# haan6/fm-for-online-recommendation

Measured on AMD Instinct MI355X. Metric: samples/sec online-FM (Criteo-39-field, k=16) FTRL-proximal, higher is better.
Workload: dtype f32

## Files before the change

### fm-for-online-recommendation_amd/csrc/fmx_common.h

```cpp
#pragma once
#include <hip/hip_runtime.h>
#include <hip/hip_ext.h>

#include <cstdarg>
#include <cstdio>
#include <cstdlib>
#include <cstring>
#include <atomic>
#include <mutex>

#include "fmx.h"

#pragma clang fp contract(off)

namespace fmxd {
extern thread_local char g_err[512];
int fail(int code, const char *fmt, ...);
int check_launch(const char *what);

struct Tune {
  int wpb_fwd = 4, wpb_upd = 2;
  int sort_e = 0;
  int inline_fixup = 1;
  int online_persistent = 1;
  int afm_online_persistent = 1;
  int afm_pair_online_persistent = 1;
  int sort_ahead = 16;
  int mlp_chain = 1;
  int sort_chunked = 1;
};
Tune &tune();

constexpr int FMX_COMM_SLOTS = 4;
struct Comm {
  int rank = 0, world = 1, n_blocks = 1;
  bool force = false;
  int block_count[FMX_COMM_MAX_WORLD] = {0}, block_first[FMX_COMM_MAX_WORLD] = {0};
  void *main = nullptr, *pf = nullptr;
  hipStream_t pf_stream = nullptr;
  hipEvent_t fork = nullptr, ready[FMX_COMM_SLOTS] = {nullptr}, free_[FMX_COMM_SLOTS] = {nullptr};
  bool used[FMX_COMM_SLOTS] = {false};
};
int comm_all_gather(Comm *c, int which, const void *send, void *recv, size_t count, hipStream_t st);
int comm_exchange_blocks(Comm *c, const float *send, float *recv, size_t per, hipStream_t st);

constexpr int MLP_BIG_MAX_L = 8;
struct MlpReduceArgs {
  const float *parts[MLP_BIG_MAX_L];
  int out_dim[MLP_BIG_MAX_L], in_dim[MLP_BIG_MAX_L], ldp[MLP_BIG_MAX_L];
  long long grad_off[MLP_BIG_MAX_L];
  float *grads;
  float *params;
  float lr;
  int rule;
  float *m, *v;
  float eps, c1, c2;
  int n_split[MLP_BIG_MAX_L], n_layers;
  const float *loss_b;
  float *loss_out;
  int B;
// ... 452 lines not shown
```

### fm-for-online-recommendation_amd/csrc/fmx_host.h

```cpp
#pragma once
#include <type_traits>

#include "fmx_common.h"

namespace fmxd {

struct Workspace {
  uint32_t *sorted;
  size_t sorted_stride;
  uint32_t *runs;
  int32_t *meta;
  int32_t *counter;
  float *parts;
  size_t bytes;
};

struct SortBatch {
  int n_pool = 1, first = 0, n_batches = 1;
  int64_t pool_stride = 0, sorted_stride = 0;
};

int check_table(const fmx_table_t *t);
int check_rule(const fmx_table_t *t, int rule);
int check_adam(const fmx_hyper_t *h, int rule, int64_t n_steps);
int check_sort_geometry(const fmx_table_t *t, int B);
int check_workspace(const fmx_table_t *t, int B, const void *workspace, int64_t workspace_bytes, const char *who);
int check_pair_args(const fmx_table_t *table, const fmx_hyper_t *hyper, const int32_t *idx, int64_t n_pairs, const char *count_name,
                    float margin, const char *who);
int named(int rc, const char *who);
int refuse_adaptive(int rule, const char *who);

int forward_impl(const fmx_table_t *table, const fmx_hyper_t *hyper, const int32_t *idx, const float *xv, const float *y,
                 int32_t B, int32_t loss_kind, float inv_b, const fmx_fwd_out_t *out, hipStream_t st);
int sort_impl(const fmx_table_t *table, const int32_t *idx, int32_t B, uint32_t *sorted, uint32_t *runs, int32_t *error,
              hipStream_t st, const SortBatch *mb = nullptr);
int update_impl(const fmx_table_t *table, const fmx_hyper_t *hyper, int32_t rule, const Workspace &w,
                const uint32_t *sorted, const float *xv, const float *S, const float *dz_first, const float *dz_bi, const float *gbi,
                int32_t B, const float *loss_b, float inv_b, float *loss_out, hipStream_t st, int32_t *step_counter = nullptr,
                int32_t sample_ld = 0, int32_t *err_flag = nullptr, const MlpReduceArgs *rider = nullptr);
int update_occ_impl(const fmx_table_t *table, const fmx_hyper_t *hyper, int32_t rule, const Workspace &w, const float *xv,
                    const float *dz_first, const float *occ, int32_t ld_occ, int32_t B, const float *loss_b, float inv_b,
                    float *loss_out, hipStream_t st);
int afm_pair_online_buffers(int F, int k, int kp, int t, int attn_rule, bool *moments_in_lds);
int afm_pair_online_launch(const fmx_table_t *table, const fmx_hyper_t *hyper, int32_t rule, const fmx_afm_t *afm, const int32_t *idx,
                           const float *xv, int32_t N_pairs, float margin, float *attn_grad_out, const fmx_mlp_opt_t *opt,
                           float *logit_out, float *loss_out, int32_t *error, int nb, bool moments_in_lds, hipStream_t st);

}

namespace {

inline int lpr_of(int kp) {
  switch (kp) {
    case 4: return 1;
    case 8: return 2;
    case 16: return 4;
    case 32: return 8;
    case 64: return 16;
    default: return 0;
  }
}

template <class Fn>
decltype(auto) with_lpr(int kp, Fn &&f) {
  switch (lpr_of(kp)) {
    case 1: return f(std::integral_constant<int, 1>{});
    case 2: return f(std::integral_constant<int, 2>{});
    case 4: return f(std::integral_constant<int, 4>{});
    case 8: return f(std::integral_constant<int, 8>{});
    default: return f(std::integral_constant<int, 16>{});
  }
}
// ... 40 lines not shown
inline const char *rule_name(int rule) { return rule == FMX_RULE_ADAM ? "FMX_RULE_ADAM" : "FMX_RULE_ADAGRAD"; }

inline bool mapped(const fmx_table_t *t) { return t->field_cols || t->field_base; }
inline int n_cols(const fmx_table_t *t) { return t->n_cols > 0 ? t->n_cols : t->n_fields; }
inline int n_sort_fields(const fmx_table_t *t) { return t->n_sort_fields > 0 ? t->n_sort_fields : t->n_fields; }
inline const int64_t *sort_offsets(const fmx_table_t *t) { return t->n_sort_fields > 0 ? t->sort_offsets : t->field_offsets; }
inline const int32_t *sort_cols(const fmx_table_t *t) { return t->n_sort_fields > 0 ? t->sort_cols : nullptr; }
inline int64_t max_sort_rows(const fmx_table_t *t) { return t->n_sort_fields > 0 ? t->max_sort_field_rows : t->max_field_rows; }

static_assert(sizeof(fmx_hyper_t) == 40, "hyper_for copies fmx_hyper_t field by field: add the new field to the copy");
inline fmx_hyper_t hyper_for(const fmx_hyper_t *h, int rule) {
  fmx_hyper_t r;
  memset(&r, 0, sizeof(r));
  r.lr = h->lr;
  r.eps = h->eps;
  r.alpha = h->alpha;
  r.beta = h->beta;
  r.l1 = h->l1;
  r.l2 = h->l2;
  if (rule == FMX_RULE_ADAM) {
    r.beta1 = h->beta1;
    r.beta2 = h->beta2;
    r.step = h->step;
  }
  return r;
}

inline fmx_hyper_t kernel_hyper(const fmx_hyper_t *h, int rule) {
  fmx_hyper_t r = hyper_for(h, rule);
  r.alpha = 1.0f / h->alpha;
  return r;
}

constexpr int SORT_AHEAD_MAX = 16;

inline Workspace carve(const fmx_table_t *t, int B, void *base) {
  const size_t F = (size_t)n_sort_fields(t), Bp = (size_t)fmx_sorted_width(B), tiles = Bp >> 6;
  const size_t rec = 2 * (size_t)t->kp + 4;
  const size_t o_sorted1 = align_up(F * Bp * 4, 256);
  const size_t o_runs = 2 * SORT_AHEAD_MAX * o_sorted1;
  const size_t o_meta = o_runs + (Bp >= 2 * SORT_CHUNK ? SORT_AHEAD_MAX * o_sorted1 : 0);
  const size_t o_counter = o_meta + align_up(F * tiles * 2 * 4, 256);
  const size_t o_parts = o_counter + 256;
  Workspace w;
  char *p = static_cast<char *>(base);
  w.sorted = reinterpret_cast<uint32_t *>(p);
  w.sorted_stride = o_sorted1 / 4;
  w.runs = reinterpret_cast<uint32_t *>(p + o_runs);
  w.meta = reinterpret_cast<int32_t *>(p + o_meta);
  w.counter = reinterpret_cast<int32_t *>(p + o_counter);
  w.parts = reinterpret_cast<float *>(p + o_parts);
  w.bytes = o_parts + align_up(F * tiles * 2 * rec * 4, 256);
  return w;
}

}
```

### fm-for-online-recommendation_amd/csrc/fmx_kernels.hip

```cpp

#include <cmath>

#include "fmx_host.h"

namespace fmxd {

thread_local char g_err[512] = "";

int fail(int code, const char *fmt, ...) {
  va_list ap;
  va_start(ap, fmt);
  vsnprintf(g_err, sizeof(g_err), fmt, ap);
  va_end(ap);
  return code;
}

int check_launch(const char *what) {
  hipError_t e = hipGetLastError();
  if (e != hipSuccess) return fail(FMX_ERR_LAUNCH, "%s: %s", what, hipGetErrorString(e));
  return FMX_OK;
}

}

// ... 455 lines not shown
                (long long)workspace_bytes, (long long)need, B, n_sort_fields(t));
  return FMX_OK;
}

int named(int rc, const char *who) {
  if (rc != FMX_OK && !strstr(g_err, who)) {
    char msg[sizeof(g_err)];
    snprintf(msg, sizeof(msg), "%s", g_err);
    snprintf(g_err, sizeof(g_err), "%s: %s", who, msg);
  }
  return rc;
}

int check_pair_args(const fmx_table_t *table, const fmx_hyper_t *hyper, const int32_t *idx, int64_t n_pairs, const char *count_name,
                    float margin, const char *who) {
  if (!table) return fail(FMX_ERR_ARG, "%s: table is null", who);
  if (int rc = check_table(table)) return named(rc, who);
  if (!hyper) return fail(FMX_ERR_ARG, "%s: hyper is null", who);
  if (!idx) return fail(FMX_ERR_ARG, "%s: idx is null", who);
  if (n_pairs < 1) return fail(FMX_ERR_ARG, "%s: %s = %lld must be >= 1", who, count_name, (long long)n_pairs);
  if (!(margin >= 0.f) || !std::isfinite(margin)) return fail(FMX_ERR_ARG, "%s: margin = %g must be finite and >= 0", who, (double)margin);
  if (mapped(table))
    return fail(FMX_ERR_UNSUPPORTED, "%s: tables whose fields are pieces of index columns (field_cols / field_base) are not taken", who);
  return FMX_OK;
}

Tune &tune() {
  static Tune t = [] {
    Tune x;
    if (const char *e = getenv("FMX_WPB_FWD")) x.wpb_fwd = atoi(e);
    if (const char *e = getenv("FMX_WPB_UPD")) x.wpb_upd = atoi(e);
    if (const char *e = getenv("FMX_SORT_E")) x.sort_e = atoi(e);
    if (const char *e = getenv("FMX_SORT_AHEAD")) x.sort_ahead = atoi(e);
    if (const char *e = getenv("FMX_ONLINE_PERSISTENT")) x.online_persistent = atoi(e);
    if (const char *e = getenv("FMX_INLINE_FIXUP")) x.inline_fixup = atoi(e);
    if (const char *e = getenv("FMX_SORT_CHUNKED")) x.sort_chunked = atoi(e);
    if (const char *e = getenv("FMX_MLP_CHAIN")) x.mlp_chain = atoi(e);
    auto ok = [](int v) { return v == 1 || v == 2 || v == 4; };
    if (!ok(x.wpb_fwd)) x.wpb_fwd = 4;
    if (!ok(x.wpb_upd)) x.wpb_upd = 2;
    return x;
  }();
  return t;
}
}
namespace {

struct Side {
  hipStream_t stream = nullptr;
  hipStream_t main = nullptr;
  hipEvent_t fork = nullptr, sorted[2] = {nullptr, nullptr}, consumed[2] = {nullptr, nullptr};
  hipEvent_t user_fork = nullptr, user_join = nullptr;
};

Side *side_for_current_device() {
  static std::mutex mu;
  static Side sides[64];
  int dev = 0;
  if (hipGetDevice(&dev) != hipSuccess || dev < 0 || dev >= 64) return nullptr;
  std::lock_guard<std::mutex> lock(mu);
  Side &sd = sides[dev];
  if (!sd.stream) {
    int lo = 0, hi = 0;
    (void)hipDeviceGetStreamPriorityRange(&lo, &hi);
    if (hipStreamCreateWithPriority(&sd.stream, hipStreamNonBlocking, lo) != hipSuccess) return nullptr;
    if (hipStreamCreateWithPriority(&sd.main, hipStreamNonBlocking, hi) != hipSuccess) return nullptr;
    bool ok = hipEventCreateWithFlags(&sd.fork, hipEventDisableTiming) == hipSuccess &&
              hipEventCreateWithFlags(&sd.user_fork, hipEventDisableTiming) == hipSuccess &&
              hipEventCreateWithFlags(&sd.user_join, hipEventDisableTiming) == hipSuccess;
    for (int i = 0; i < 2 && ok; ++i) {
      ok = hipEventCreateWithFlags(&sd.sorted[i], hipEventDisableTiming) == hipSuccess &&
           hipEventCreateWithFlags(&sd.consumed[i], hipEventDisableTiming) == hipSuccess;
    }
    if (!ok) return nullptr;
  }
  return &sd;
}

constexpr int OVERLAP_MIN_BATCH = 512;

template <int LPR, int NPASS, bool MAPPED = false, bool PAIR = false>
void launch_forward_np(const FwdArgs &a, int layout, hipStream_t st) {
  const int wpb = PAIR && tune().wpb_fwd < 2 ? 2 : tune().wpb_fwd;
  const dim3 grid((a.B + wpb - 1) / wpb), block(64 * wpb);
  if (layout == FMX_LAYOUT_FTRL) hipLaunchKernelGGL((k_fm_forward<LPR, FMX_LAYOUT_FTRL, NPASS, MAPPED, PAIR>), grid, block, 0, st, a);
  else hipLaunchKernelGGL((k_fm_forward<LPR, FMX_LAYOUT_WEIGHTS, NPASS, MAPPED, PAIR>), grid, block, 0, st, a);
}

template <int LPR, bool PAIR = false>
void launch_forward(const FwdArgs &a, int layout, hipStream_t st) {
  const int slots = WAVE / LPR;
  const int np = (a.F + slots - 1) / slots;
  if constexpr (!PAIR) {
    if (a.fcols || a.fbase) {
      launch_forward_np<LPR, 0, true>(a, layout, st);
      return;
    }
  }
  if (!with_one_of<1, 2, 3, 4>(np, [&](auto NP) { launch_forward_np<LPR, NP, false, PAIR>(a, layout, st); }))
    launch_forward_np<LPR, 0, false, PAIR>(a, layout, st);
}

template <int E>
void launch_sort(SortArgs a, hipStream_t st) {
  const int threads = a.Bp / E;
  uint32_t lds = (uint32_t)(a.Bp * sizeof(uint32_t));
  if (a.Bp <= RADIX_SMALL_WIDTH && threads >= 64) {
    a.small_bits = RADIX_SMALL_BITS;
    const uint32_t need = (uint32_t)radix_small_lds_bytes(a.Bp, threads);
// ... 82 lines not shown

int sort_pool(const fmx_table_t *table, const int32_t *idx_pool, int n_pool, int B, int first_step, int n, const Workspace &w,
              uint32_t *sorted, int32_t *error, hipStream_t st) {
  SortBatch mb;
  mb.n_pool = n_pool;
  mb.first = first_step % n_pool;
  mb.n_batches = n;
  mb.pool_stride = (int64_t)B * (int64_t)n_cols(table);
  mb.sorted_stride = (int64_t)w.sorted_stride;
  return sort_impl(table, idx_pool, B, sorted, w.runs, error, st, &mb);
}

struct Detour {
  Side *sd;
  hipStream_t user, st;
  Detour(Side *side, hipStream_t stream) : sd(stream == nullptr ? side : nullptr), user(stream), st(stream) {
    if (!sd) return;
    (void)hipEventRecord(sd->user_fork, user);
    st = sd->main;
    (void)hipStreamWaitEvent(st, sd->user_fork, 0);
  }
  ~Detour() {
    if (!sd) return;
    (void)hipEventRecord(sd->user_join, st);
    (void)hipStreamWaitEvent(user, sd->user_join, 0);
  }
  Detour(const Detour &) = delete;
  Detour &operator=(const Detour &) = delete;
};

template <class BeforeUpdate, class Update>
int pool_loop(const fmx_table_t *table, const int32_t *idx_pool, const float *y_pool, int n_pool, int B, int n_steps,
              const Workspace &w, int32_t *error, hipStream_t stream, BeforeUpdate &&before_update, Update &&update) {
  Side *sd = (B >= OVERLAP_MIN_BATCH && n_steps > 0) ? side_for_current_device() : nullptr;
  const Detour detour(sd, stream);
  const hipStream_t st = detour.st;
  const size_t F = (size_t)n_cols(table);
  int ahead = tune().sort_ahead;
  if (ahead < 1) ahead = 1;
  if (ahead > SORT_AHEAD_MAX) ahead = SORT_AHEAD_MAX;
  auto group_size = [&](int g, int first_step) {
    int n = g == 0 ? 4 : ahead;
    if (n > ahead) n = ahead;
    if (n > n_steps - first_step) n = n_steps - first_step;
    return n;
  };
  auto sort_group = [&](int g, int first_step, int n, hipStream_t where) -> int {
    return sort_pool(table, idx_pool, n_pool, B, first_step, n, w, w.sorted + (size_t)(g & 1) * ahead * w.sorted_stride, error, where);
  };
  int rc = FMX_OK;
  if (sd) {
    (void)hipEventRecord(sd->fork, st);
    (void)hipStreamWaitEvent(sd->stream, sd->fork, 0);
    rc = sort_group(0, 0, group_size(0, 0), sd->stream);
    (void)hipEventRecord(sd->sorted[0], sd->stream);
  }
  int first_step = 0;
  for (int g = 0; first_step < n_steps && rc == FMX_OK; ++g) {
    const int n = group_size(g, first_step);
    const int next_first = first_step + n;
    if (!sd) rc = sort_group(g, first_step, n, st);
    for (int i = 0; i < n && rc == FMX_OK; ++i) {
      const int s = first_step + i, j = s % n_pool;
      rc = before_update(s, idx_pool + (size_t)j * B * F, y_pool ? y_pool + (size_t)j * B : nullptr, st);
      if (sd && i == 0) (void)hipStreamWaitEvent(st, sd->sorted[g & 1], 0);
      if (rc == FMX_OK) rc = update(s, w.sorted + ((size_t)(g & 1) * ahead + i) * w.sorted_stride, st);
      if (sd && i == 0 && next_first < n_steps && rc == FMX_OK) {
        if (g >= 1) (void)hipStreamWaitEvent(sd->stream, sd->consumed[(g + 1) & 1], 0);
        rc = sort_group(g + 1, next_first, group_size(g + 1, next_first), sd->stream);
        (void)hipEventRecord(sd->sorted[(g + 1) & 1], sd->stream);
      }
    }
    if (sd) (void)hipEventRecord(sd->consumed[g & 1], st);
    first_step = next_first;
  }
  return rc;
}

FwdArgs fill_fwd(const fmx_table_t *table, const fmx_hyper_t *hyper, const int32_t *idx, const float *xv, const float *y,
                 int32_t B, int32_t loss_kind, float inv_b, const fmx_fwd_out_t *out) {
  FwdArgs a;
  a.ldS = out->sample_ld > 0 ? out->sample_ld : table->kp;
  a.ld1 = out->sample_ld > 0 ? out->sample_ld : 1;
  a.rows = table->rows;
  a.foff = table->field_offsets;
  a.bias = table->bias;
  a.idx = idx;
  a.xv = xv;
  a.y = y;
  a.out = *out;
  a.h = kernel_hyper(hyper, -1);
  a.B = B;
  a.F = table->n_fields;
  a.Fc = n_cols(table);
  a.fcols = table->field_cols;
  a.fbase = table->field_base;
  a.kp = table->kp;
  a.stride = table->row_stride;
  a.zoff = table->z_offset;
  a.loss_kind = loss_kind;
  a.inv_b = inv_b;
  a.margin = 0.f;
// ... 81 lines not shown
    return fail(FMX_ERR_SHAPE, "sample_ld=%d must be 0 or a multiple of 4 that is >= kp", out->sample_ld);
  return FMX_OK;
}

int check_step_args(const fmx_table_t *table, const fmx_hyper_t *hyper, int32_t rule, int32_t loss_kind, int32_t B,
                    const void *workspace, const fmx_fwd_out_t *fwd) {
  if (int rc = check_table(table)) return rc;
  if (int rc = check_rule(table, rule)) return rc;
  if (int rc = check_sort_geometry(table, B)) return rc;
  if (!hyper || !workspace) return fail(FMX_ERR_ARG, "null hyper / workspace");
  if (int rc = check_adam(hyper, rule, 1)) return rc;
  if (!aligned16(workspace)) return fail(FMX_ERR_ALIGN, "workspace must be 16-byte aligned");
  if (!fwd || !fwd->S || !fwd->dz || !fwd->loss) return fail(FMX_ERR_ARG, "fwd->S, fwd->loss, fwd->dz are required");
  if (!aligned16(fwd->S) || !aligned16(fwd->dz) || !aligned16(fwd->loss))
    return fail(FMX_ERR_ALIGN, "fwd->S, fwd->dz and fwd->loss must be 16-byte aligned");
  if (loss_kind != FMX_LOSS_BCE_LOGITS && loss_kind != FMX_LOSS_BCE_SIGMOID) return fail(FMX_ERR_ARG, "a step needs a loss");
  return FMX_OK;
}

#include "fmx_pair.inc"

}

extern "C" {

int fmx_version(void) { return FMX_VERSION; }

int fmx_set_option(const char *name, int value) {
  if (!name) return fail(FMX_ERR_ARG, "fmx_set_option: null name");
  Tune &t = tune();
  int *slot = nullptr;
  if (!strcmp(name, "inline_fixup")) slot = &t.inline_fixup;
  else if (!strcmp(name, "sort_ahead")) slot = &t.sort_ahead;
  else if (!strcmp(name, "online_persistent")) slot = &t.online_persistent;
  else if (!strcmp(name, "afm_online_persistent")) slot = &t.afm_online_persistent;
  else if (!strcmp(name, "afm_pair_online_persistent")) slot = &t.afm_pair_online_persistent;
  else if (!strcmp(name, "sort_chunked")) slot = &t.sort_chunked;
  else if (!strcmp(name, "mlp_chain")) slot = &t.mlp_chain;
  else return fail(FMX_ERR_ARG, "fmx_set_option: unknown option '%s'", name);
  const int old = *slot;
  *slot = value;
  return old;
}

const char *fmx_last_error_string(void) { return g_err; }

int fmx_sorted_width(int B) {
  int w = 64;
  while (w < B && w < (1 << 30)) w <<= 1;
  return w;
}

int fmx_sorted_bbits(int B) {
  int w = fmx_sorted_width(B), bits = 0;
  while ((1 << bits) < w) ++bits;
  return bits;
}

int64_t fmx_workspace_bytes(const fmx_table_t *table, int32_t B) {
  if (check_table(table) != FMX_OK) return FMX_ERR_ARG;
  if (B < 1) return fail(FMX_ERR_ARG, "B must be >= 1");
  return (int64_t)carve(table, B, nullptr).bytes;
}

int fmx_fm_forward(const fmx_table_t *table, const fmx_hyper_t *hyper, const int32_t *idx, const float *xv,
                   const float *y, int32_t B, int32_t loss_kind, float inv_b, const fmx_fwd_out_t *out,
// ... 111 lines not shown
  if (fwd->sample_ld != 0) return fail(FMX_ERR_ARG, "%s: dense forward outputs only (sample_ld = 0)", who);
  if (!fm_term && (!fwd->sfirst || (opt ? table->layout == FMX_LAYOUT_FTRL : table->layout != FMX_LAYOUT_WEIGHTS)))
    return fail(FMX_ERR_UNSUPPORTED, "%s: fm_term = 0 (NFM) needs fwd->sfirst and a table in the weights%s layout", who, opt ? " or the moments" : "");
  if (!idx_pool || (!pair && !y_pool) || n_pool < 1 || n_steps < 0 || B < 1) return fail(FMX_ERR_ARG, "%s: bad pool / step count", who);
  if (opt) {
    if (int rc = check_adam(hyper, rule, n_steps)) return rc;
    if (int rc = mlp_opt_check(mlp, B, mlp_workspace, mlp_workspace_bytes, grads, opt, n_steps, who)) return rc;
  }
  if (pair && !opt) {
    const int64_t need = fmx_mlp_section_workspace_bytes(mlp, B);
    if (need < 0) return fail(FMX_ERR_UNSUPPORTED, "%s: needs 1 <= layers <= %d, k >= 1, hidden >= 1", who, MLP_BIG_MAX_L);
    if (mlp_workspace_bytes < need)
      return fail(FMX_ERR_SHAPE, "%s: the MLP workspace holds %lld bytes, fmx_mlp_section_workspace_bytes asks for %lld", who,
                  (long long)mlp_workspace_bytes, (long long)need);
  }
  if (mlp->k > table->kp) return fail(FMX_ERR_SHAPE, "%s: the MLP reads k=%d columns of a bi of kp=%d", who, mlp->k, table->kp);
  if (!aligned16(gbi) || !aligned16(dz)) return fail(FMX_ERR_ALIGN, "dz and gbi must be 16-byte aligned");
  if (int rc = check_sort_geometry(table, B)) return rc;
  if (int rc = check_workspace(table, B, workspace, workspace_bytes, who)) return rc;
  const Workspace w = carve(table, B, workspace);
  MlpReduceArgs red;
  auto before_update = [&](int s, const int32_t *idx, const float *y, hipStream_t st) -> int {
    int rc = forward_impl(table, hyper, idx, nullptr, nullptr, B, FMX_LOSS_NONE, inv_b, fwd, st);
    if (rc == FMX_OK && !fm_term) {
      hipLaunchKernelGGL(k_first_plus_bias, dim3((B + 255) / 256), dim3(256), 0, st, fwd->logit, fwd->sfirst, table->bias, B);
      rc = check_launch("fmx_deepfm_stream (k_first_plus_bias)");
    }
    if (rc == FMX_OK)
      rc = mlp_section_deferred_reduce(mlp, loss_kind, fwd->bi, table->kp, fwd->logit, y, B, inv_b, mlp_workspace, nullptr, dz, gbi, table->kp,
                                       grads, opt ? 0.f : lr_mlp, loss_out ? loss_out + s : nullptr, st, &red, who, pair_margin);
    if (rc == FMX_OK && opt) mlp_reduce_set_opt(red, *opt, opt->step + s + 1);
    return rc;
  };
  auto update = [&](int s, const uint32_t *sorted, hipStream_t st) {
    fmx_hyper_t hs = hyper_for(hyper, rule);
    hs.step += s;
    return update_impl(table, &hs, rule, w, sorted, nullptr, fwd->S, dz, fm_term ? dz : nullptr, gbi, B, nullptr, inv_b, nullptr, st, nullptr, 0,
                       fwd->error, &red);
  };
  return pool_loop(table, idx_pool, y_pool, n_pool, B, n_steps, w, fwd->error, static_cast<hipStream_t>(stream), before_update, update);
}

int fmx_deepfm_stream(const fmx_table_t *table, const fmx_hyper_t *hyper, int32_t rule, const fmx_mlp_t *mlp, int32_t loss_kind, int32_t fm_term,
                      const int32_t *idx_pool, const float *y_pool, int32_t n_pool, int32_t B, float inv_b, int32_t n_steps,
                      void *workspace, int64_t workspace_bytes, void *mlp_workspace, const fmx_fwd_out_t *fwd, float *dz, float *gbi,
                      float *grads, float lr_mlp, float *loss_out, fmx_stream_t stream) {
  return deepfm_stream_impl(table, hyper, rule, mlp, loss_kind, fm_term, idx_pool, y_pool, n_pool, B, inv_b, n_steps, workspace, workspace_bytes,
                            mlp_workspace, 0, fwd, dz, gbi, grads, lr_mlp, nullptr, loss_out, stream, "fmx_deepfm_stream");
}

int fmx_deepfm_stream_opt(const fmx_table_t *table, const fmx_hyper_t *hyper, int32_t rule, const fmx_mlp_t *mlp, int32_t loss_kind,
                          int32_t fm_term, const int32_t *idx_pool, const float *y_pool, int32_t n_pool, int32_t B, float inv_b,
                          int32_t n_steps, void *workspace, int64_t workspace_bytes, void *mlp_workspace, int64_t mlp_workspace_bytes,
                          const fmx_fwd_out_t *fwd, float *dz, float *gbi, float *grads, const fmx_mlp_opt_t *opt, float *loss_out,
                          fmx_stream_t stream) {
  if (!opt) return fail(FMX_ERR_ARG, "fmx_deepfm_stream_opt: opt is null");
  return deepfm_stream_impl(table, hyper, rule, mlp, loss_kind, fm_term, idx_pool, y_pool, n_pool, B, inv_b, n_steps, workspace, workspace_bytes,
                            mlp_workspace, mlp_workspace_bytes, fwd, dz, gbi, grads, 0.f, opt, loss_out, stream, "fmx_deepfm_stream_opt");
}

int fmx_deepfm_pair_stream(const fmx_table_t *table, const fmx_hyper_t *hyper, int32_t rule, const fmx_mlp_t *mlp, int32_t fm_term,
                           const int32_t *idx_pool, int32_t n_pool, int32_t B_pairs, float margin, float inv_b, int32_t n_steps,
                           void *workspace, int64_t workspace_bytes, void *mlp_workspace, int64_t mlp_workspace_bytes,
                           const fmx_fwd_out_t *fwd, float *dz, float *gbi, float *grads, float lr_mlp, const fmx_mlp_opt_t *opt,
                           float *loss_out, fmx_stream_t stream) {
  const char *who = "fmx_deepfm_pair_stream";
  if (int rc = check_pair_args(table, hyper, idx_pool, B_pairs, "B_pairs", margin, who)) return rc;
  if (int rc = check_sort_geometry(table, pair_rows(B_pairs))) return rc;
  if (n_pool < 1) return fail(FMX_ERR_ARG, "%s: n_pool = %d must be >= 1", who, n_pool);
  if (n_steps < 0) return fail(FMX_ERR_ARG, "%s: n_steps = %d must be >= 0", who, n_steps);
  return named(deepfm_stream_impl(table, hyper, rule, mlp, FMX_LOSS_NONE, fm_term, idx_pool, nullptr, n_pool, 2 * B_pairs, inv_b, n_steps, workspace,
// ... 75 lines not shown
  (void)hipEventRecord(c->free_[slot], st);
  c->used[slot] = true;
  return FMX_OK;
}

int fmx_fm_step(const fmx_table_t *table, const fmx_hyper_t *hyper, int32_t rule, int32_t loss_kind,
                const int32_t *idx, const float *xv, const float *y, int32_t B, float inv_b, void *workspace, int64_t workspace_bytes,
                const fmx_fwd_out_t *fwd, float *loss_out, fmx_stream_t stream) {
  if (int rc = check_step_args(table, hyper, rule, loss_kind, B, workspace, fwd)) return rc;
  if (!idx || !y) return fail(FMX_ERR_ARG, "fmx_fm_step: idx and y are required");
  hipStream_t st = static_cast<hipStream_t>(stream);
  if (int rc = check_workspace(table, B, workspace, workspace_bytes, "fmx_fm_step")) return rc;
  const Workspace w = carve(table, B, workspace);
  if (int rc = sort_impl(table, idx, B, w.sorted, w.runs, fwd->error, st)) return rc;
  if (int rc = forward_impl(table, hyper, idx, xv, y, B, loss_kind, inv_b, fwd, st)) return rc;
  return update_impl(table, hyper, rule, w, w.sorted, xv, fwd->S, fwd->dz, fwd->dz, nullptr, B, fwd->loss, inv_b, loss_out, st,
                     nullptr, fwd->sample_ld, fwd->error);
}

int fmx_fm_stream(const fmx_table_t *table, const fmx_hyper_t *hyper, int32_t rule, int32_t loss_kind,
                  const int32_t *idx_pool, const float *y_pool, int32_t n_pool, int32_t B, float inv_b,
                  int32_t n_steps, void *workspace, int64_t workspace_bytes, const fmx_fwd_out_t *fwd, float *loss_out, float *kernel_ms,
                  fmx_stream_t stream) {
  if (int rc = check_step_args(table, hyper, rule, loss_kind, B, workspace, fwd)) return rc;
  if (!idx_pool || !y_pool || n_pool < 1 || n_steps < 0) return fail(FMX_ERR_ARG, "fmx_fm_stream: bad pool / step count");
  if (int rc = check_adam(hyper, rule, n_steps)) return rc;
  hipStream_t st = static_cast<hipStream_t>(stream);
  if (int rc = check_workspace(table, B, workspace, workspace_bytes, "fmx_fm_stream")) return rc;
  const Workspace w = carve(table, B, workspace);
  if (!kernel_ms) {
    auto forward = [&](int, const int32_t *idx, const float *y, hipStream_t st) {
      return forward_impl(table, hyper, idx, nullptr, y, B, loss_kind, inv_b, fwd, st);
    };
    auto update = [&](int s, const uint32_t *sorted, hipStream_t st) {
      fmx_hyper_t hs = hyper_for(hyper, rule);
      hs.step += s;
      return update_impl(table, &hs, rule, w, sorted, nullptr, fwd->S, fwd->dz, fwd->dz, nullptr, B, fwd->loss, inv_b,
                         loss_out ? loss_out + s : nullptr, st, nullptr, fwd->sample_ld, fwd->error);
    };
    return pool_loop(table, idx_pool, y_pool, n_pool, B, n_steps, w, fwd->error, st, forward, update);
  }

  const int REP = 8, n_ev = 5;
  const int n_groups = (n_steps + REP - 1) / REP;
  const size_t F = (size_t)n_cols(table);
  const size_t region = align_up((size_t)B * table->kp + 2 * (size_t)B, 64);
  float *tmp = nullptr;
  hipEvent_t *ev = nullptr;
  int rc = FMX_OK;
  {
    const Detour detour(st == nullptr ? side_for_current_device() : nullptr, st);
    st = detour.st;
    if (n_groups > 0 && hipMalloc(&tmp, REP * region * sizeof(float)) != hipSuccess)
      return fail(FMX_ERR_LAUNCH, "hipMalloc (measuring mode)");
    ev = new hipEvent_t[(size_t)n_groups * n_ev];
    for (int i = 0; i < n_groups * n_ev; ++i) (void)hipEventCreate(&ev[i]);
    for (int g = 0; g < n_groups && rc == FMX_OK; ++g) {
      const int first = g * REP, n = (n_steps - first) < REP ? (n_steps - first) : REP;
      hipEvent_t *e = ev + (size_t)g * n_ev;
      (void)hipEventRecord(e[0], st);
      rc = sort_pool(table, idx_pool, n_pool, B, first, n, w, w.sorted, fwd->error, st);
      (void)hipEventRecord(e[1], st);
      for (int r = 0; r < n && rc == FMX_OK; ++r) {
        const int j = (first + r) % n_pool;
        fmx_fwd_out_t fr = *fwd;
        fr.S = tmp + (size_t)r * region;
        fr.dz = fr.S + (size_t)B * table->kp;
        fr.loss = fr.dz + B;
        fr.sample_ld = 0;
        rc = forward_impl(table, hyper, idx_pool + (size_t)j * B * F, nullptr, y_pool + (size_t)j * B, B, loss_kind, inv_b, &fr, st);
      }
// ... 86 lines not shown
```

### fm-for-online-recommendation_amd/csrc/fmx_pair.inc

```

inline int32_t pair_rows(int32_t B_pairs) { return B_pairs > INT32_MAX / 2 ? INT32_MAX : 2 * B_pairs; }

int check_pair_out(const fmx_table_t *table, const fmx_fwd_out_t *out, const char *name, bool step, const char *who) {
  if (!out) return fail(FMX_ERR_ARG, "%s: %s is null", who, name);
  if (step) {
    if (!out->S) return fail(FMX_ERR_ARG, "%s: %s->S is required", who, name);
    if (!out->loss) return fail(FMX_ERR_ARG, "%s: %s->loss is required", who, name);
    if (!out->dz) return fail(FMX_ERR_ARG, "%s: %s->dz is required", who, name);
    if (!aligned16(out->dz) || !aligned16(out->loss)) return fail(FMX_ERR_ALIGN, "%s: %s->dz and %s->loss must be 16-byte aligned", who, name, name);
  }
  if ((out->S && !aligned16(out->S)) || (out->bi && !aligned16(out->bi)))
    return fail(FMX_ERR_ALIGN, "%s: %s->S and %s->bi must be 16-byte aligned", who, name, name);
  if (out->sample_ld != 0 && (out->sample_ld < table->kp || out->sample_ld % 4))
    return fail(FMX_ERR_SHAPE, "%s: %s->sample_ld = %d must be 0 or a multiple of 4 that is >= kp", who, name, out->sample_ld);
  return FMX_OK;
}

int pair_forward_impl(const fmx_table_t *table, const fmx_hyper_t *hyper, const int32_t *idx, const float *xv, int32_t B2, float margin,
                      float inv_b, const fmx_fwd_out_t *out, hipStream_t st) {
  FwdArgs a = fill_fwd(table, hyper, idx, xv, nullptr, B2, FMX_LOSS_NONE, inv_b, out);
  a.margin = margin;
  with_lpr(table->kp, [&](auto LPR) { launch_forward<LPR, true>(a, table->layout, st); });
  return check_launch("k_fm_forward (pair)");
}
// ... 12 lines not shown
  if (int rc = check_pair_args(table, hyper, idx, B_pairs, "B_pairs", margin, who)) return rc;
  if (int rc = check_rule(table, rule)) return named(rc, who);
  if (int rc = check_adam(hyper, rule, n_steps)) return named(rc, who);
  if (int rc = check_pair_out(table, fwd, "fwd", true, who)) return rc;
  if (int rc = check_sort_geometry(table, pair_rows(B_pairs))) return rc;
  return check_workspace(table, pair_rows(B_pairs), workspace, workspace_bytes, who);
}

int pair_step_call(const fmx_table_t *table, const fmx_hyper_t *hyper, int32_t rule, const int32_t *idx, const float *xv, int32_t B_pairs,
                   float margin, float inv_b, void *workspace, int64_t workspace_bytes, const fmx_fwd_out_t *fwd, float *loss_out,
                   hipStream_t st) {
  if (int rc = check_pair_step(table, hyper, rule, idx, B_pairs, margin, workspace, workspace_bytes, fwd, 1, "fmx_fm_pair_step")) return rc;
  const int32_t B2 = 2 * B_pairs;
  const Workspace w = carve(table, B2, workspace);
  if (int rc = sort_impl(table, idx, B2, w.sorted, w.runs, fwd->error, st)) return rc;
  if (int rc = pair_forward_impl(table, hyper, idx, xv, B2, margin, inv_b, fwd, st)) return rc;
  return update_impl(table, hyper, rule, w, w.sorted, xv, fwd->S, fwd->dz, fwd->dz, nullptr, B2, fwd->loss, inv_b, loss_out, st, nullptr,
                     fwd->sample_ld, fwd->error);
}

int pair_stream_call(const fmx_table_t *table, const fmx_hyper_t *hyper, int32_t rule, const int32_t *idx_pool, int32_t n_pool,
                     int32_t B_pairs, float margin, float inv_b, int32_t n_steps, void *workspace, int64_t workspace_bytes,
                     const fmx_fwd_out_t *fwd, float *loss_out, hipStream_t st) {
  const char *who = "fmx_fm_pair_stream";
  if (int rc = check_pair_step(table, hyper, rule, idx_pool, B_pairs, margin, workspace, workspace_bytes, fwd, n_steps > 0 ? n_steps : 0, who))
    return rc;
  if (n_pool < 1) return fail(FMX_ERR_ARG, "%s: n_pool = %d must be >= 1", who, n_pool);
  if (n_steps < 0) return fail(FMX_ERR_ARG, "%s: n_steps = %d must be >= 0", who, n_steps);
  const int32_t B2 = 2 * B_pairs;
  const Workspace w = carve(table, B2, workspace);
  auto forward = [&](int, const int32_t *idx, const float *, hipStream_t s_) {
    return pair_forward_impl(table, hyper, idx, nullptr, B2, margin, inv_b, fwd, s_);
  };
  auto update = [&](int s, const uint32_t *sorted, hipStream_t s_) {
    fmx_hyper_t hs = hyper_for(hyper, rule);
    hs.step += s;
    return update_impl(table, &hs, rule, w, sorted, nullptr, fwd->S, fwd->dz, fwd->dz, nullptr, B2, fwd->loss, inv_b,
                       loss_out ? loss_out + s : nullptr, s_, nullptr, fwd->sample_ld, fwd->error);
  };
  return pool_loop(table, idx_pool, nullptr, n_pool, B2, n_steps, w, fwd->error, st, forward, update);
}
```

### fm-for-online-recommendation_amd/csrc/fmx_update.hip

```cpp

#include "fmx_host.h"

namespace {

__device__ __forceinline__ void st_sc1(float *p, float v) { __hip_atomic_store(p, v, __ATOMIC_RELAXED, __HIP_MEMORY_SCOPE_AGENT); }
typedef float v4f __attribute__((ext_vector_type(4)));
__device__ __forceinline__ void st_sc1_4(float *p, float4 v) {
  const v4f x = {v.x, v.y, v.z, v.w};
  asm volatile("global_store_dwordx4 %0, %1, off sc1\n\ts_nop 1" ::"v"(p), "v"(x) : "memory");
}
__device__ __forceinline__ void store_part_sc1(float *rec, int q, int kp, float4 cV, float4 cA, float cw) {
  st_sc1_4(rec + 4 * q, cV);
  st_sc1_4(rec + kp + 4 * q, cA);
  if (q == 0) st_sc1(rec + 2 * kp, cw);
}

struct UpdArgs {
  float *rows;
  const int64_t *foff;
  float *bias;
  const uint32_t *sorted;
  float *parts;
  int32_t *meta;
  const float *xv;
  const float *S;
  const float *dz_first;
  const float *dz_bi;
  const float *gbi;
  const float *loss_b;
  float *loss_out;
  int32_t *step_counter;
  fmx_hyper_t h;
  int32_t B, F, Bp, bbits, kp, stride, zoff;
  int32_t ldS, ld1;
  int32_t ldG;
  const int32_t *cols;
  const int32_t *fcols;
  int32_t Fx;
  float *red;
  uint32_t seq;
  int32_t *error;
  float inv_b;
};

constexpr int LEAD_NONE = 0, LEAD_CLOSES = 1, LEAD_THROUGH = 2;

constexpr int RED_SLICE = 4096;
__host__ __device__ inline int red_slices(int B) { return (B + RED_SLICE - 1) / RED_SLICE; }

template <int LAYOUT, int RULE>
__device__ __forceinline__ void apply_bias_and_loss(const UpdArgs &a, float db, float ls) {
  constexpr bool MOM = LAYOUT == FMX_LAYOUT_MOMENTS;
  float b0 = a.bias[0], b1 = LAYOUT != FMX_LAYOUT_WEIGHTS ? a.bias[1] : 0.f, b2 = MOM ? a.bias[2] : 0.f;
  bias_step<LAYOUT, RULE>(b0, b1, b2, db, a.h);
  st4(a.bias, b0);
  if (LAYOUT == FMX_LAYOUT_FTRL || (MOM && RULE == FMX_RULE_ADAM)) st4(a.bias + 1, b1);
  if (MOM) st4(a.bias + 2, b2);
  if (a.loss_b && a.loss_out) {
    int i = 0;
    if (a.step_counter) {
      i = *a.step_counter;
      *a.step_counter = i + 1;
    }
    a.loss_out[i] = ls * a.inv_b;
  }
}

template <int LAYOUT, int RULE>
__device__ void finish_bias_and_loss(const UpdArgs &a, int R, bool poll) {
  __shared__ float part[2 * 16];
  const int t = threadIdx.x;
  bool failed = false;
  if (t < R) {
    const v4f *src = reinterpret_cast<const v4f *>(a.red) + t;
    v4f g = {0.f, 0.f, 0.f, 0.f};
// ... 69 lines not shown
  do {                                                                                                              \
    unsigned long long t_;                                                                                          \
    asm volatile("s_memrealtime %0\n\ts_waitcnt lgkmcnt(0)" : "=s"(t_) : "v"(dep_) : "memory");                      \
    if (lane == 0 && gt < 8192) g_upd_stamps[(size_t)gt * 6 + (slot_)] = t_;                                         \
  } while (0)
#else
#define FMX_STAMP(slot_, dep_) do {} while (0)
#endif

template <int LPR, int LAYOUT, int RULE, bool HAS_GBI, bool INL, bool OCC = false>
__device__ __forceinline__ void update_body(const UpdArgs &a, const int blk) {
  constexpr int SLOTS = WAVE / LPR;
  constexpr int EPG = LPR;
  constexpr int REC = 2 * LPR * 4 + 4;
  constexpr bool PREFETCH_ROWS = EPG <= 4;
  using CA = CoefA<HAS_GBI>;
  const int n_red = red_slices(a.B);
  if (blk < n_red) {
    bias_and_loss<LAYOUT, RULE, INL>(a, blk);
    return;
  }
  const int lane = threadIdx.x & 63;
  const int slot = lane / LPR, q = lane % LPR;
  const int kp = LPR * 4;
  const int tiles_per_field = a.Bp >> 6;
  const int gt = (blk - n_red) * (blockDim.x >> 6) + (threadIdx.x >> 6);
  if (gt >= a.F * tiles_per_field) return;
  const int f = gt / tiles_per_field;
  const int base = (gt - f * tiles_per_field) << 6;
  const uint32_t *sf = a.sorted + (size_t)f * a.Bp;
  const int bbits = a.bbits;
  const uint32_t bmask = (1u << bbits) - 1u;
  const int e0 = base + slot * EPG;
  FMX_STAMP(0, lane);

  uint32_t c[EPG];
  if constexpr (EPG % 4 == 0) {
#pragma unroll
    for (int j = 0; j < EPG; j += 4) {
      const uint4 t = *reinterpret_cast<const uint4 *>(sf + e0 + j);
      c[j] = t.x;
      c[j + 1] = t.y;
      c[j + 2] = t.z;
      c[j + 3] = t.w;
    }
  } else {
#pragma unroll
    for (int j = 0; j < EPG; ++j) c[j] = sf[e0 + j];
  }
  const uint32_t kprev = (e0 == 0 ? SENT : sf[e0 - 1]) >> bbits;
  const uint32_t knext = (e0 + EPG < a.Bp ? sf[e0 + EPG] : SENT) >> bbits;
  const uint32_t tile_prevkey = (base == 0 ? SENT : sf[base - 1]) >> bbits;
  const size_t row0 = (size_t)a.foff[f];
  float *part = a.parts + (size_t)gt * 2 * REC;

  uint32_t k[EPG];
  bool val[EPG], tail[EPG];
#pragma unroll
  for (int j = 0; j < EPG; ++j) {
    k[j] = c[j] >> bbits;
    val[j] = c[j] != SENT;
  }
#pragma unroll
  for (int j = 0; j < EPG; ++j) tail[j] = val[j] && (k[j] != (j + 1 < EPG ? k[j + 1] : knext));
  FMX_STAMP(1, k[0] + knext + kprev + tile_prevkey);

// ... 303 lines not shown
  RowRegs r;
  if (lane < LPR) r = load_row<LAYOUT, RULE>(rp, q, kp, a.zoff);
  int m = 0;
  for (int j0 = 1; t + j0 < tiles_per_field; j0 += 64) {
    const int tj = t + j0 + lane;
    const int st = j0 == 1 ? st0 : (tj < tiles_per_field ? a.meta[((size_t)f * tiles_per_field + tj) * 2] : LEAD_NONE);
    const unsigned long long stop = __ballot(st != LEAD_THROUGH);
    if (stop != 0ull) {
      const int pos = __ffsll((long long)stop) - 1;
      const int st_pos = __shfl(st, pos);
      m = j0 + pos - (st_pos == LEAD_CLOSES ? 0 : 1);
      break;
    }
    m = j0 + 63;
  }
  if (t + m >= tiles_per_field) m = tiles_per_field - 1 - t;
  float4 aV = splat(0.f), aA = splat(0.f);
  float aw = 0.f;
  for (int j = slot; j <= m; j += SLOTS) {
    const float *rec = j == 0 ? a.parts + ((size_t)gt * 2 + 1) * REC : a.parts + (size_t)(gt + j) * 2 * REC;
    aV = aV + *reinterpret_cast<const float4 *>(rec + 4 * q);
    aA = aA + *reinterpret_cast<const float4 *>(rec + kp + 4 * q);
    aw += rec[2 * kp];
  }
#pragma unroll
  for (int mm = LPR; mm < WAVE; mm <<= 1) {
    aV = aV + shfl_xor4(aV, mm);
    aA = aA + shfl_xor4(aA, mm);
    aw += __shfl_xor(aw, mm);
  }
  if (lane < LPR) update_row<LAYOUT, RULE>(rp, q, kp, a.zoff, r, aV, aA, aw, a.h);
}

bool is_capturing(hipStream_t st) {
  if (!st) return false;
  hipStreamCaptureStatus cs = hipStreamCaptureStatusNone;
  return hipStreamIsCapturing(st, &cs) == hipSuccess && cs != hipStreamCaptureStatusNone;
}

template <int LPR, bool HAS_GBI, bool INL>
void launch_update(const UpdArgs &a, int rule, hipStream_t st) {
  const int tiles = a.F * (a.Bp >> 6);
  const int wpb = tune().wpb_upd;
  const dim3 grid((tiles + wpb - 1) / wpb + red_slices(a.B)), block(64 * wpb);
  with_rule(rule, [&](auto LAYOUT, auto RULE) { hipLaunchKernelGGL((k_fm_update<LPR, LAYOUT, RULE, HAS_GBI, INL>), grid, block, 0, st, a); });
}

template <int LPR>
void launch_update_rider(const UpdArgs &a, int rule, const MlpReduceArgs &r, hipStream_t st) {
  const int tiles = a.F * (a.Bp >> 6);
  const int wpb = tune().wpb_upd;
  const int n_upd = (tiles + wpb - 1) / wpb + red_slices(a.B), per = mlp_reduce_blocks_per_layer(r, 64 * wpb);
  const dim3 grid(n_upd + per * r.n_layers), block(64 * wpb);
  with_rule(rule, [&](auto LAYOUT, auto RULE) {
    hipLaunchKernelGGL((k_fm_update_rider<LPR, LAYOUT, RULE, true>), grid, block, 0, st, a, r, n_upd, per);
  });
}

template <int LPR>
void launch_fixup(const UpdArgs &a, int rule, hipStream_t st) {
  const int tiles = a.F * (a.Bp >> 6);
  const int wpb = tune().wpb_upd;
  const dim3 grid((tiles + wpb - 1) / wpb + (red_slices(a.B) > 1 ? 1 : 0)), block(64 * wpb);
  with_rule(rule, [&](auto LAYOUT, auto RULE) { hipLaunchKernelGGL((k_fm_fixup<LPR, LAYOUT, RULE>), grid, block, 0, st, a); });
}

template <int LPR>
void launch_update_pair(const UpdArgs &a, int rule, bool has_gbi, hipStream_t st) {
  if (tune().inline_fixup && !is_capturing(st)) {
    if (has_gbi) launch_update<LPR, true, true>(a, rule, st);
    else launch_update<LPR, false, true>(a, rule, st);
    return;
  }
  if (has_gbi) launch_update<LPR, true, false>(a, rule, st);
  else launch_update<LPR, false, false>(a, rule, st);
  launch_fixup<LPR>(a, rule, st);
}

template <int LPR>
void launch_update_occ_pair(const UpdArgs &a, int rule, hipStream_t st) {
  const int tiles = a.F * (a.Bp >> 6);
  const int wpb = tune().wpb_upd;
  const dim3 grid((tiles + wpb - 1) / wpb + red_slices(a.B)), block(64 * wpb);
  const bool inl = tune().inline_fixup && !is_capturing(st);
  with_rule(rule, [&](auto LAYOUT, auto RULE) {
    if (inl) hipLaunchKernelGGL((k_fm_update_occ<LPR, LAYOUT, RULE, true>), grid, block, 0, st, a);
    else hipLaunchKernelGGL((k_fm_update_occ<LPR, LAYOUT, RULE, false>), grid, block, 0, st, a);
  });
  if (!inl) launch_fixup<LPR>(a, rule, st);
}

UpdArgs fill_upd(const fmx_table_t *table, const fmx_hyper_t *hyper, const Workspace &w, const uint32_t *sorted,
                 const float *xv, const float *S, const float *dz_first, const float *dz_bi, const float *gbi, int32_t B,
                 const float *loss_b, float inv_b, float *loss_out, int32_t *step_counter, int32_t sample_ld,
                 int32_t *err_flag) {
  UpdArgs a;
  a.ldS = sample_ld > 0 ? sample_ld : table->kp;
  a.ld1 = sample_ld > 0 ? sample_ld : 1;
  a.ldG = sample_ld > 0 ? sample_ld : table->kp;
  static std::atomic<uint32_t> launch_seq{1};
  a.seq = launch_seq.fetch_add(1) & 0x0FFFFFFFu;
  if (a.seq == 0) a.seq = launch_seq.fetch_add(1) & 0x0FFFFFFFu;
  a.error = err_flag;
  a.rows = table->rows;
  a.foff = sort_offsets(table);
  a.cols = sort_cols(table);
  a.Fx = n_cols(table);
  a.fcols = table->field_cols;
  a.bias = table->bias;
  a.sorted = sorted;
  a.parts = w.parts;
  a.meta = w.meta;
  a.red = reinterpret_cast<float *>(w.counter);
  a.xv = xv;
  a.S = S;
  a.dz_first = dz_first;
  a.dz_bi = dz_bi;
  a.gbi = gbi;
  a.loss_b = loss_b;
  a.loss_out = loss_out;
  a.step_counter = step_counter;
  a.h = kernel_hyper(hyper, -1);
  a.B = B;
  a.F = n_sort_fields(table);
  a.Bp = fmx_sorted_width(B);
  a.bbits = fmx_sorted_bbits(B);
  a.kp = table->kp;
  a.stride = table->row_stride;
  a.zoff = table->z_offset;
  a.inv_b = inv_b;
  return a;
}

}

namespace fmxd {

int update_impl(const fmx_table_t *table, const fmx_hyper_t *hyper, int32_t rule, const Workspace &w,
                const uint32_t *sorted, const float *xv,
                const float *S, const float *dz_first, const float *dz_bi, const float *gbi, int32_t B,
                const float *loss_b, float inv_b, float *loss_out, hipStream_t st,
                int32_t *step_counter, int32_t sample_ld, int32_t *err_flag, const MlpReduceArgs *rider) {
  UpdArgs a = fill_upd(table, hyper, w, sorted, xv, S, dz_first, dz_bi, gbi, B, loss_b, inv_b, loss_out, step_counter,
                       sample_ld, err_flag);
  if (rule == FMX_RULE_ADAM)
    adam_consts(hyper->lr, hyper->beta1, hyper->beta2, hyper->step + 1, a.h.lr, a.h.beta1, a.h.beta2);
  if (rider) {
    if (gbi != nullptr && tune().inline_fixup && !is_capturing(st)) {
      with_lpr(table->kp, [&](auto LPR) { launch_update_rider<LPR>(a, rule, *rider, st); });
      return check_launch("k_fm_update_rider");
    }
    mlp_launch_reduce(*rider, st);
  }
  with_lpr(table->kp, [&](auto LPR) { launch_update_pair<LPR>(a, rule, gbi != nullptr, st); });
  return check_launch("k_fm_update / k_fm_fixup");
}

int update_occ_impl(const fmx_table_t *table, const fmx_hyper_t *hyper, int32_t rule, const Workspace &w, const float *xv,
                    const float *dz_first, const float *occ, int32_t ld_occ, int32_t B, const float *loss_b, float inv_b,
                    float *loss_out, hipStream_t st) {
  UpdArgs a = fill_upd(table, hyper, w, w.sorted, xv, nullptr, dz_first, nullptr, occ, B, loss_b, inv_b, loss_out, nullptr, 0,
                       nullptr);
  a.ldG = ld_occ;
  if (rule == FMX_RULE_ADAM) adam_consts(hyper->lr, hyper->beta1, hyper->beta2, hyper->step + 1, a.h.lr, a.h.beta1, a.h.beta2);
  with_lpr(table->kp, [&](auto LPR) { launch_update_occ_pair<LPR>(a, rule, st); });
  return check_launch("k_fm_update_occ / k_fm_fixup");
}

}

#ifdef FMX_STAMPS
extern "C" int fmx_debug_update_stamps(unsigned long long *host_out) {
  return hipMemcpyFromSymbol(host_out, HIP_SYMBOL(g_upd_stamps), sizeof(unsigned long long) * 8192 * 6) == hipSuccess ? FMX_OK : FMX_ERR_LAUNCH;
}
#endif
```

Before: 199.6 million.

## Replace cross-stream sort event wait with device-side spin gate in update kernel

The update kernel that consumes a pre-sorted group no longer waits for the sort stream through a hipStreamWaitEvent. The sort stream now publishes a sequence number to a device word after each sort group, and the inline-fixup update kernel spins on that word with relaxed atomic loads and sleeps, then issues an acquire fence. This is meant to remove the host/driver cross-stream dependency latency so the update can launch immediately. The cost is spinning wavefronts that may occupy CUs while the sort runs, a possible deadlock if the sort kernel cannot be scheduled, handled by a timeout that sets an error, and an extra tiny publish kernel per group.

```diff
diff --git a/fm-for-online-recommendation_amd/csrc/fmx_common.h b/fm-for-online-recommendation_amd/csrc/fmx_common.h
--- a/fm-for-online-recommendation_amd/csrc/fmx_common.h
+++ b/fm-for-online-recommendation_amd/csrc/fmx_common.h
@@ -26,6 +26,7 @@
   int afm_online_persistent = 1;
   int afm_pair_online_persistent = 1;
   int sort_ahead = 16;
+  int sort_gate = 1;
   int mlp_chain = 1;
   int sort_chunked = 1;
 };
diff --git a/fm-for-online-recommendation_amd/csrc/fmx_host.h b/fm-for-online-recommendation_amd/csrc/fmx_host.h
--- a/fm-for-online-recommendation_amd/csrc/fmx_host.h
+++ b/fm-for-online-recommendation_amd/csrc/fmx_host.h
@@ -20,6 +20,11 @@
   int64_t pool_stride = 0, sorted_stride = 0;
 };
 
+struct SortGate {
+  const uint64_t *word;
+  uint64_t seq;
+};
+
 int check_table(const fmx_table_t *t);
 int check_rule(const fmx_table_t *t, int rule);
 int check_adam(const fmx_hyper_t *h, int rule, int64_t n_steps);
@@ -37,7 +42,8 @@
 int update_impl(const fmx_table_t *table, const fmx_hyper_t *hyper, int32_t rule, const Workspace &w,
                 const uint32_t *sorted, const float *xv, const float *S, const float *dz_first, const float *dz_bi, const float *gbi,
                 int32_t B, const float *loss_b, float inv_b, float *loss_out, hipStream_t st, int32_t *step_counter = nullptr,
-                int32_t sample_ld = 0, int32_t *err_flag = nullptr, const MlpReduceArgs *rider = nullptr);
+                int32_t sample_ld = 0, int32_t *err_flag = nullptr, const MlpReduceArgs *rider = nullptr,
+                const SortGate *gate = nullptr);
 int update_occ_impl(const fmx_table_t *table, const fmx_hyper_t *hyper, int32_t rule, const Workspace &w, const float *xv,
                     const float *dz_first, const float *occ, int32_t ld_occ, int32_t B, const float *loss_b, float inv_b,
                     float *loss_out, hipStream_t st);
@@ -144,6 +150,12 @@
   return r;
 }
 
+inline bool is_capturing(hipStream_t st) {
+  if (!st) return false;
+  hipStreamCaptureStatus cs = hipStreamCaptureStatusNone;
+  return hipStreamIsCapturing(st, &cs) == hipSuccess && cs != hipStreamCaptureStatusNone;
+}
+
 constexpr int SORT_AHEAD_MAX = 16;
 
 inline Workspace carve(const fmx_table_t *t, int B, void *base) {
diff --git a/fm-for-online-recommendation_amd/csrc/fmx_kernels.hip b/fm-for-online-recommendation_amd/csrc/fmx_kernels.hip
--- a/fm-for-online-recommendation_amd/csrc/fmx_kernels.hip
+++ b/fm-for-online-recommendation_amd/csrc/fmx_kernels.hip
@@ -511,6 +511,7 @@
     if (const char *e = getenv("FMX_WPB_UPD")) x.wpb_upd = atoi(e);
     if (const char *e = getenv("FMX_SORT_E")) x.sort_e = atoi(e);
     if (const char *e = getenv("FMX_SORT_AHEAD")) x.sort_ahead = atoi(e);
+    if (const char *e = getenv("FMX_SORT_GATE")) x.sort_gate = atoi(e);
     if (const char *e = getenv("FMX_ONLINE_PERSISTENT")) x.online_persistent = atoi(e);
     if (const char *e = getenv("FMX_INLINE_FIXUP")) x.inline_fixup = atoi(e);
     if (const char *e = getenv("FMX_SORT_CHUNKED")) x.sort_chunked = atoi(e);
@@ -530,9 +531,22 @@
   hipStream_t main = nullptr;
   hipEvent_t fork = nullptr, sorted[2] = {nullptr, nullptr}, consumed[2] = {nullptr, nullptr};
   hipEvent_t user_fork = nullptr, user_join = nullptr;
+  uint64_t *gate = nullptr;
 };
-
-Side *side_for_current_device() {
+constexpr int GATE_STRIDE = 16;
+
+bool side_gate_alloc(Side &sd) {
+  uint64_t *p = nullptr;
+  if (hipMalloc(&p, 2 * GATE_STRIDE * sizeof(uint64_t)) != hipSuccess) return false;
+  if (hipMemsetAsync(p, 0, 2 * GATE_STRIDE * sizeof(uint64_t), sd.stream) != hipSuccess || hipStreamSynchronize(sd.stream) != hipSuccess) {
+    (void)hipFree(p);
+    return false;
+  }
+  sd.gate = p;
+  return true;
+}
+
+Side *side_for_current_device(hipStream_t user = nullptr) {
   static std::mutex mu;
   static Side sides[64];
   int dev = 0;
@@ -553,7 +567,21 @@
     }
     if (!ok) return nullptr;
   }
+  if (!sd.gate && !is_capturing(user) && !side_gate_alloc(sd)) return nullptr;
   return &sd;
+}
+
+__global__ void k_sort_publish(uint64_t *word, uint64_t seq) {
+  __hip_atomic_store(word, seq, __ATOMIC_RELAXED, __HIP_MEMORY_SCOPE_AGENT);
+}
+
+uint64_t publish_sorted(Side *sd, int half) {
+  static std::mutex mu;
+  static uint64_t next = 1;
+  std::lock_guard<std::mutex> lock(mu);
+  const uint64_t seq = next++;
+  hipLaunchKernelGGL(k_sort_publish, dim3(1), dim3(1), 0, sd->stream, sd->gate + (size_t)half * GATE_STRIDE, seq);
+  return seq;
 }
 
 constexpr int OVERLAP_MIN_BATCH = 512;
@@ -702,9 +730,11 @@
 template <class BeforeUpdate, class Update>
 int pool_loop(const fmx_table_t *table, const int32_t *idx_pool, const float *y_pool, int n_pool, int B, int n_steps,
               const Workspace &w, int32_t *error, hipStream_t stream, BeforeUpdate &&before_update, Update &&update) {
-  Side *sd = (B >= OVERLAP_MIN_BATCH && n_steps > 0) ? side_for_current_device() : nullptr;
+  Side *sd = (B >= OVERLAP_MIN_BATCH && n_steps > 0) ? side_for_current_device(stream) : nullptr;
   const Detour detour(sd, stream);
   const hipStream_t st = detour.st;
+  const bool gated = sd && sd->gate && tune().sort_gate && tune().inline_fixup && !is_capturing(st);
+  uint64_t gate_seq[2] = {0, 0};
   const size_t F = (size_t)n_cols(table);
   int ahead = tune().sort_ahead;
   if (ahead < 1) ahead = 1;
@@ -733,11 +763,14 @@
     for (int i = 0; i < n && rc == FMX_OK; ++i) {
       const int s = first_step + i, j = s % n_pool;
       rc = before_update(s, idx_pool + (size_t)j * B * F, y_pool ? y_pool + (size_t)j * B : nullptr, st);
-      if (sd && i == 0) (void)hipStreamWaitEvent(st, sd->sorted[g & 1], 0);
-      if (rc == FMX_OK) rc = update(s, w.sorted + ((size_t)(g & 1) * ahead + i) * w.sorted_stride, st);
+      const SortGate gate{gated ? sd->gate + (size_t)(g & 1) * GATE_STRIDE : nullptr, gate_seq[g & 1]};
+      const bool at_gate = gated && i == 0 && g >= 1;
+      if (sd && i == 0 && !at_gate) (void)hipStreamWaitEvent(st, sd->sorted[g & 1], 0);
+      if (rc == FMX_OK) rc = update(s, w.sorted + ((size_t)(g & 1) * ahead + i) * w.sorted_stride, at_gate ? &gate : nullptr, st);
       if (sd && i == 0 && next_first < n_steps && rc == FMX_OK) {
         if (g >= 1) (void)hipStreamWaitEvent(sd->stream, sd->consumed[(g + 1) & 1], 0);
         rc = sort_group(g + 1, next_first, group_size(g + 1, next_first), sd->stream);
+        if (gated && rc == FMX_OK) gate_seq[(g + 1) & 1] = publish_sorted(sd, (g + 1) & 1);
         (void)hipEventRecord(sd->sorted[(g + 1) & 1], sd->stream);
       }
     }
@@ -885,6 +918,7 @@
   int *slot = nullptr;
   if (!strcmp(name, "inline_fixup")) slot = &t.inline_fixup;
   else if (!strcmp(name, "sort_ahead")) slot = &t.sort_ahead;
+  else if (!strcmp(name, "sort_gate")) slot = &t.sort_gate;
   else if (!strcmp(name, "online_persistent")) slot = &t.online_persistent;
   else if (!strcmp(name, "afm_online_persistent")) slot = &t.afm_online_persistent;
   else if (!strcmp(name, "afm_pair_online_persistent")) slot = &t.afm_pair_online_persistent;
@@ -1062,11 +1096,11 @@
     if (rc == FMX_OK && opt) mlp_reduce_set_opt(red, *opt, opt->step + s + 1);
     return rc;
   };
-  auto update = [&](int s, const uint32_t *sorted, hipStream_t st) {
+  auto update = [&](int s, const uint32_t *sorted, const SortGate *gate, hipStream_t st) {
     fmx_hyper_t hs = hyper_for(hyper, rule);
     hs.step += s;
     return update_impl(table, &hs, rule, w, sorted, nullptr, fwd->S, dz, fm_term ? dz : nullptr, gbi, B, nullptr, inv_b, nullptr, st, nullptr, 0,
-                       fwd->error, &red);
+                       fwd->error, &red, gate);
   };
   return pool_loop(table, idx_pool, y_pool, n_pool, B, n_steps, w, fwd->error, static_cast<hipStream_t>(stream), before_update, update);
 }
@@ -1208,11 +1242,11 @@
     auto forward = [&](int, const int32_t *idx, const float *y, hipStream_t st) {
       return forward_impl(table, hyper, idx, nullptr, y, B, loss_kind, inv_b, fwd, st);
     };
-    auto update = [&](int s, const uint32_t *sorted, hipStream_t st) {
+    auto update = [&](int s, const uint32_t *sorted, const SortGate *gate, hipStream_t st) {
       fmx_hyper_t hs = hyper_for(hyper, rule);
       hs.step += s;
       return update_impl(table, &hs, rule, w, sorted, nullptr, fwd->S, fwd->dz, fwd->dz, nullptr, B, fwd->loss, inv_b,
-                         loss_out ? loss_out + s : nullptr, st, nullptr, fwd->sample_ld, fwd->error);
+                         loss_out ? loss_out + s : nullptr, st, nullptr, fwd->sample_ld, fwd->error, nullptr, gate);
     };
     return pool_loop(table, idx_pool, y_pool, n_pool, B, n_steps, w, fwd->error, st, forward, update);
   }
diff --git a/fm-for-online-recommendation_amd/csrc/fmx_pair.inc b/fm-for-online-recommendation_amd/csrc/fmx_pair.inc
--- a/fm-for-online-recommendation_amd/csrc/fmx_pair.inc
+++ b/fm-for-online-recommendation_amd/csrc/fmx_pair.inc
@@ -68,11 +68,11 @@
   auto forward = [&](int, const int32_t *idx, const float *, hipStream_t s_) {
     return pair_forward_impl(table, hyper, idx, nullptr, B2, margin, inv_b, fwd, s_);
   };
-  auto update = [&](int s, const uint32_t *sorted, hipStream_t s_) {
+  auto update = [&](int s, const uint32_t *sorted, const SortGate *gate, hipStream_t s_) {
     fmx_hyper_t hs = hyper_for(hyper, rule);
     hs.step += s;
     return update_impl(table, &hs, rule, w, sorted, nullptr, fwd->S, fwd->dz, fwd->dz, nullptr, B2, fwd->loss, inv_b,
-                       loss_out ? loss_out + s : nullptr, s_, nullptr, fwd->sample_ld, fwd->error);
+                       loss_out ? loss_out + s : nullptr, s_, nullptr, fwd->sample_ld, fwd->error, nullptr, gate);
   };
   return pool_loop(table, idx_pool, nullptr, n_pool, B2, n_steps, w, fwd->error, st, forward, update);
 }
diff --git a/fm-for-online-recommendation_amd/csrc/fmx_update.hip b/fm-for-online-recommendation_amd/csrc/fmx_update.hip
--- a/fm-for-online-recommendation_amd/csrc/fmx_update.hip
+++ b/fm-for-online-recommendation_amd/csrc/fmx_update.hip
@@ -41,6 +41,8 @@
   uint32_t seq;
   int32_t *error;
   float inv_b;
+  const uint64_t *gate;
+  uint64_t gate_seq;
 };
 
 constexpr int LEAD_NONE = 0, LEAD_CLOSES = 1, LEAD_THROUGH = 2;
@@ -176,6 +178,21 @@
   const int bbits = a.bbits;
   const uint32_t bmask = (1u << bbits) - 1u;
   const int e0 = base + slot * EPG;
+  if (INL && a.gate) {
+    bool open = false;
+    for (int spin = 0; spin <= (1 << 20) && !open; ++spin) {
+      uint64_t v = 0;
+      if (lane == 0) v = __hip_atomic_load(a.gate, __ATOMIC_RELAXED, __HIP_MEMORY_SCOPE_AGENT);
+      v = ((uint64_t)__builtin_amdgcn_readfirstlane((uint32_t)(v >> 32)) << 32) | __builtin_amdgcn_readfirstlane((uint32_t)v);
+      open = v >= a.gate_seq;
+      if (!open) __builtin_amdgcn_s_sleep(1);
+    }
+    if (!open) {
+      if (lane == 0 && a.error) *a.error = 2;
+      return;
+    }
+    __builtin_amdgcn_fence(__ATOMIC_ACQUIRE, "agent");
+  }
   FMX_STAMP(0, lane);
 
   uint32_t c[EPG];
@@ -545,12 +562,6 @@
   if (lane < LPR) update_row<LAYOUT, RULE>(rp, q, kp, a.zoff, r, aV, aA, aw, a.h);
 }
 
-bool is_capturing(hipStream_t st) {
-  if (!st) return false;
-  hipStreamCaptureStatus cs = hipStreamCaptureStatusNone;
-  return hipStreamIsCapturing(st, &cs) == hipSuccess && cs != hipStreamCaptureStatusNone;
-}
-
 template <int LPR, bool HAS_GBI, bool INL>
 void launch_update(const UpdArgs &a, int rule, hipStream_t st) {
   const int tiles = a.F * (a.Bp >> 6);
@@ -580,7 +591,7 @@
 
 template <int LPR>
 void launch_update_pair(const UpdArgs &a, int rule, bool has_gbi, hipStream_t st) {
-  if (tune().inline_fixup && !is_capturing(st)) {
+  if (a.gate || (tune().inline_fixup && !is_capturing(st))) {
     if (has_gbi) launch_update<LPR, true, true>(a, rule, st);
     else launch_update<LPR, false, true>(a, rule, st);
     return;
@@ -642,6 +653,8 @@
   a.stride = table->row_stride;
   a.zoff = table->z_offset;
   a.inv_b = inv_b;
+  a.gate = nullptr;
+  a.gate_seq = 0;
   return a;
 }
 
@@ -653,13 +666,17 @@
                 const uint32_t *sorted, const float *xv,
                 const float *S, const float *dz_first, const float *dz_bi, const float *gbi, int32_t B,
                 const float *loss_b, float inv_b, float *loss_out, hipStream_t st,
-                int32_t *step_counter, int32_t sample_ld, int32_t *err_flag, const MlpReduceArgs *rider) {
+                int32_t *step_counter, int32_t sample_ld, int32_t *err_flag, const MlpReduceArgs *rider, const SortGate *gate) {
   UpdArgs a = fill_upd(table, hyper, w, sorted, xv, S, dz_first, dz_bi, gbi, B, loss_b, inv_b, loss_out, step_counter,
                        sample_ld, err_flag);
+  if (gate) {
+    a.gate = gate->word;
+    a.gate_seq = gate->seq;
+  }
   if (rule == FMX_RULE_ADAM)
     adam_consts(hyper->lr, hyper->beta1, hyper->beta2, hyper->step + 1, a.h.lr, a.h.beta1, a.h.beta2);
   if (rider) {
-    if (gbi != nullptr && tune().inline_fixup && !is_capturing(st)) {
+    if (gbi != nullptr && (gate || (tune().inline_fixup && !is_capturing(st)))) {
       with_lpr(table->kp, [&](auto LPR) { launch_update_rider<LPR>(a, rule, *rider, st); });
       return check_launch("k_fm_update_rider");
     }
```

After: 192.8 million. -3.4%, worse.
